# Kamino666/video_features

Hardware: AMD Instinct MI355X
Metric: frames/sec CLIP-ViT-B/32 uni_12 (higher is better)
Workload: dtype bf16; 1 GPU; model=CLIP-ViT-B/32, global_batch=256, seq_len=12, resolution=224, parallelism=dp1

## Files before the change

video_features_amd/models/clip_vit.py:

```python
from __future__ import annotations

from dataclasses import dataclass

import torch
from torch import nn

from .. import ops


@dataclass
class ViTConfig:
    input_resolution: int = 224
    patch_size: int = 32
    width: int = 768
    layers: int = 12
    heads: int = 12
    output_dim: int = 512


VIT_B32 = ViTConfig(patch_size=32)
VIT_B16 = ViTConfig(patch_size=16)


class LayerNorm(nn.LayerNorm):
    def forward(self, x: torch.Tensor) -> torch.Tensor:
        return ops.layer_norm(x, self.weight, self.bias, self.eps)


class MultiheadSelfAttention(nn.Module):
    def __init__(self, width: int, heads: int):
        super().__init__()
        self.heads = heads
        self.head_dim = width // heads
        self.qkv = nn.Linear(width, 3 * width)
        self.proj = nn.Linear(width, width)

    def forward(self, x: torch.Tensor) -> torch.Tensor:
        o = ops.mhsa_fused(self.qkv(x), self.heads)
        return self.proj(o)


class MLP(nn.Module):
    def __init__(self, width: int):
        super().__init__()
        self.c_fc = nn.Linear(width, 4 * width)
        self.c_proj = nn.Linear(4 * width, width)

    def forward(self, x: torch.Tensor) -> torch.Tensor:
        h = ops.linear_act(x, self.c_fc.weight, self.c_fc.bias, 'quick_gelu')
        return self.c_proj(h)


class ResidualAttentionBlock(nn.Module):
    def __init__(self, width: int, heads: int):
        super().__init__()
        self.ln_1 = LayerNorm(width)
        self.attn = MultiheadSelfAttention(width, heads)
        self.ln_2 = LayerNorm(width)
        self.mlp = MLP(width)

    def forward(self, x: torch.Tensor) -> torch.Tensor:
        x = x + self.attn(self.ln_1(x))
        x = x + self.mlp(self.ln_2(x))
        return x


class VisionTransformer(nn.Module):
    def __init__(self, cfg: ViTConfig = VIT_B32):
        super().__init__()
        self.cfg = cfg
        w = cfg.width
        self.conv1 = nn.Conv2d(3, w, kernel_size=cfg.patch_size,
                               stride=cfg.patch_size, bias=False)
        n_patches = (cfg.input_resolution // cfg.patch_size) ** 2
        scale = w ** -0.5
        self.class_embedding = nn.Parameter(scale * torch.randn(w))
        self.positional_embedding = nn.Parameter(
            scale * torch.randn(n_patches + 1, w))
        self.ln_pre = LayerNorm(w)
        self.blocks = nn.ModuleList(
            [ResidualAttentionBlock(w, cfg.heads) for _ in range(cfg.layers)])
        self.ln_post = LayerNorm(w)
        self.proj = nn.Parameter(scale * torch.randn(w, cfg.output_dim))

    def _patch_embed(self, x: torch.Tensor) -> torch.Tensor:
        if x.is_cuda:
            t = x.shape[0]
            p = self.cfg.patch_size
            g = x.shape[-1] // p
            xp = x.reshape(t, 3, g, p, g, p).permute(0, 2, 4, 1, 3, 5)
            xp = xp.reshape(t, g * g, 3 * p * p)
            w = self.conv1.weight.reshape(self.cfg.width, -1)
            return xp @ w.t()
        x = self.conv1(x)
        return x.flatten(2).transpose(1, 2)

    def forward(self, x: torch.Tensor) -> torch.Tensor:
        x = self._patch_embed(x)
        cls = self.class_embedding.to(x.dtype).expand(x.shape[0], 1, -1)
        x = torch.cat([cls, x], dim=1)
        x = x + self.positional_embedding.to(x.dtype)
        x = self.ln_pre(x)
        delta, res = None, x
        for blk in self.blocks:
            if delta is None:
                y1, s1 = blk.ln_1(res), res
            else:
                y1, s1 = ops.layer_norm_residual(delta, res, blk.ln_1.weight,
                                                 blk.ln_1.bias, blk.ln_1.eps)
            a = blk.attn(y1)
            y2, s2 = ops.layer_norm_residual(a, s1, blk.ln_2.weight,
                                             blk.ln_2.bias, blk.ln_2.eps)
            delta, res = blk.mlp(y2), s2
        x = delta + res
        x = self.ln_post(x[:, 0, :])
        return x @ self.proj.to(x.dtype)

    def encode_image(self, x: torch.Tensor) -> torch.Tensor:
        return self.forward(x)


def build_clip_vit(feature_type: str) -> VisionTransformer:
    if feature_type in ('CLIP-ViT-B/32', 'CLIP4CLIP-ViT-B-32'):
        return VisionTransformer(VIT_B32)
    if feature_type == 'CLIP-ViT-B/16':
        return VisionTransformer(VIT_B16)
    raise ValueError(f'unknown CLIP feature type {feature_type!r}')
```

video_features_amd/ops/__init__.py:

```python
from __future__ import annotations

import math
import os
from typing import Optional

import torch

_ext = None
_ext_err: Optional[str] = None


def _env_flag(name: str) -> bool:
    return os.environ.get(name, '').strip().lower() not in (
        '', '0', 'false', 'no', 'off')


def _load_extension():
    global _ext, _ext_err
    if _ext is not None or _ext_err is not None:
        return _ext
    try:
        from . import _vfa_hip
        _ext = _vfa_hip
    except ImportError as e:
        _ext_err = str(e)
    return _ext


def hip_available() -> bool:
    return _load_extension() is not None


def _use_hip(t: torch.Tensor) -> bool:
    if not t.is_cuda:
        return False
    if _env_flag('VFA_FORCE_TORCH_OPS'):
        return False
    ext = _load_extension()
    if ext is None:
        raise RuntimeError(
            'Tensor is on GPU but the VFA HIP extension is not built '
            f'(import error: {_ext_err}). Build it in-tree with '
            '`python setup.py build_ext --inplace` (PYTORCH_ROCM_ARCH=gfx950). '
            'Refusing to fall back to eager PyTorch on a GPU run.')
    return True


def layer_norm(x: torch.Tensor, weight: torch.Tensor, bias: torch.Tensor,
               eps: float = 1e-5) -> torch.Tensor:
    if _use_hip(x) and x.dtype in (torch.bfloat16, torch.float16, torch.float32):
        return _ext.layer_norm(x.contiguous(), weight, bias, eps)
    return torch.nn.functional.layer_norm(x, (x.shape[-1],), weight, bias, eps)


def quick_gelu(x: torch.Tensor) -> torch.Tensor:
    if _use_hip(x) and x.dtype in (torch.bfloat16, torch.float16, torch.float32):
        return _ext.quick_gelu(x.contiguous())
    return x * torch.sigmoid(1.702 * x)


def gelu(x: torch.Tensor) -> torch.Tensor:
    if _use_hip(x) and x.dtype in (torch.bfloat16, torch.float16, torch.float32):
        return _ext.gelu_tanh(x.contiguous())
    return torch.nn.functional.gelu(x, approximate='tanh')


def attention(q: torch.Tensor, k: torch.Tensor, v: torch.Tensor,
              scale: Optional[float] = None) -> torch.Tensor:
    if scale is None:
        scale = 1.0 / math.sqrt(q.shape[-1])
    if (_use_hip(q) and q.dtype in (torch.bfloat16, torch.float16, torch.float32)
            and q.shape[-2] <= 64 and q.shape[-1] <= 128):
        return _ext.mhsa(q.contiguous(), k.contiguous(), v.contiguous(),
                         float(scale))
    attn = (q @ k.transpose(-2, -1)) * scale
    attn = attn.softmax(dim=-1)
    return attn @ v


def layer_norm_residual(x: torch.Tensor, res: torch.Tensor,
                        weight: torch.Tensor, bias: torch.Tensor,
                        eps: float = 1e-5):
    if _use_hip(x) and x.dtype in (torch.bfloat16, torch.float16, torch.float32):
        y, s = _ext.layer_norm_residual(x.contiguous(), res.contiguous(),
                                        weight, bias, eps)
        return y, s
    s = x + res
    y = torch.nn.functional.layer_norm(s, (s.shape[-1],), weight, bias, eps)
    return y, s


def preprocess_u8_chw(frames_u8: torch.Tensor, mean, std,
                      bf16: bool = True) -> torch.Tensor:
    if _use_hip(frames_u8) and \
            (frames_u8.shape[1] * frames_u8.shape[2]) % 4 == 0:
        return _ext.u8_chw_norm(frames_u8.contiguous(), list(map(float, mean)),
                                list(map(float, std)), bf16)
    x = frames_u8.permute(0, 3, 1, 2).float() / 255.0
    mean_t = torch.as_tensor(mean, dtype=x.dtype, device=x.device)
    std_t = torch.as_tensor(std, dtype=x.dtype, device=x.device)
    x = (x - mean_t[:, None, None]) / std_t[:, None, None]
    return x.to(torch.bfloat16) if bf16 else x


def mhsa_fused(qkv: torch.Tensor, heads: int,
               scale: Optional[float] = None) -> torch.Tensor:
    b, n, three_e = qkv.shape
    e = three_e // 3
    d = e // heads
    if scale is None:
        scale = 1.0 / math.sqrt(d)
    if _use_hip(qkv) and qkv.dtype == torch.bfloat16 and d == 64:
        qkv5 = qkv.view(b, n, 3, heads, d)
        return _ext.flash_qkv(qkv5.contiguous(), float(scale))
    q, k, v = qkv.view(b, n, 3, heads, d).permute(2, 0, 3, 1, 4).unbind(0)
    o = attention(q.contiguous(), k.contiguous(), v.contiguous(), scale)
    return o.permute(0, 2, 1, 3).reshape(b, n, e)


def pwc_correlation(f1: torch.Tensor, f2: torch.Tensor,
                    max_disp: int = 4) -> torch.Tensor:
    if _use_hip(f1):
        return _ext.pwc_correlation(f1.contiguous(), f2.contiguous(), max_disp)
    return _pwc_correlation_torch(f1, f2, max_disp)


def _pwc_correlation_torch(f1: torch.Tensor, f2: torch.Tensor,
                           max_disp: int) -> torch.Tensor:
    b, c, h, w = f1.shape
    d = max_disp
    f2p = torch.nn.functional.pad(f2, (d, d, d, d))
    out = f1.new_empty(b, (2 * d + 1) ** 2, h, w)
    i = 0
    for dy in range(2 * d + 1):
        for dx in range(2 * d + 1):
            out[:, i] = (f1 * f2p[:, :, dy:dy + h, dx:dx + w]).mean(dim=1)
            i += 1
    return out


def bilinear_warp(x: torch.Tensor, flow: torch.Tensor) -> torch.Tensor:
    if _use_hip(x):
        return _ext.bilinear_warp(x.contiguous(), flow.contiguous())
    b, c, h, w = x.shape
    yy, xx = torch.meshgrid(
        torch.arange(h, device=x.device, dtype=x.dtype),
        torch.arange(w, device=x.device, dtype=x.dtype), indexing='ij')
    grid_x = (xx[None] + flow[:, 0]) / max(w - 1, 1) * 2 - 1
    grid_y = (yy[None] + flow[:, 1]) / max(h - 1, 1) * 2 - 1
    grid = torch.stack([grid_x, grid_y], dim=-1)
    warped = torch.nn.functional.grid_sample(x, grid, mode='bilinear',
                                             padding_mode='zeros',
                                             align_corners=True)
    mask = torch.nn.functional.grid_sample(torch.ones_like(x[:, :1]), grid,
                                           mode='bilinear', padding_mode='zeros',
                                           align_corners=True)
    return warped * (mask > 0.999).to(x.dtype)


def corr_lookup(pyramid, coords: torch.Tensor, radius: int = 4,
                nhwc: bool = False,
                out_dtype: Optional[torch.dtype] = None) -> torch.Tensor:
    if out_dtype is None:
        out_dtype = coords.dtype
    if _use_hip(coords) and radius == 4:
        return _ext.corr_lookup(list(pyramid), coords.contiguous(), nhwc,
                                out_dtype,
                                _env_flag('VFA_CORR_GMEM'))
    b, _, h, w = coords.shape
    r = radius
    cc = coords.permute(0, 2, 3, 1)
    out = []
    for lvl, corr in enumerate(pyramid):
        dx = torch.linspace(-r, r, 2 * r + 1, device=coords.device,
                            dtype=torch.float32)
        delta = torch.stack(torch.meshgrid(dx, dx, indexing='ij'), dim=-1)
        centroid = cc.reshape(b * h * w, 1, 1, 2) / (2 ** lvl)
        window = centroid + delta[None]
        sampled = grid_sample_bilinear(corr, window)
        out.append(sampled.reshape(b, h, w, -1))
    res = torch.cat(out, dim=-1).permute(0, 3, 1, 2).to(out_dtype)
    return res.contiguous(memory_format=torch.channels_last) if nhwc \
        else res.contiguous()


def convex_upsample(flow: torch.Tensor, mask: torch.Tensor,
                    nhwc: bool = False) -> torch.Tensor:
    if _use_hip(flow):
        return _ext.convex_upsample(flow, mask, nhwc)
    b, _, h, w = flow.shape
    m = (0.25 * mask.float()).view(b, 1, 9, 8, 8, h, w).softmax(dim=2)
    up = torch.nn.functional.unfold(8 * flow.float(), 3, padding=1)
    up = up.view(b, 2, 9, 1, 1, h, w)
    up = (m * up).sum(dim=2)
    return up.permute(0, 1, 4, 2, 5, 3).reshape(b, 2, 8 * h, 8 * w) \
        .to(flow.dtype)


def gru_zr(zr: torch.Tensor, hx: torch.Tensor, rhx: torch.Tensor,
           nhwc: bool = False) -> torch.Tensor:
    c = zr.shape[1] // 2
    if _use_hip(zr):
        return _ext.gru_zr(zr, hx, rhx, nhwc)
    z = torch.sigmoid(zr[:, :c])
    r = torch.sigmoid(zr[:, c:])
    rhx[:, :c] = r * hx[:, :c]
    return z


def gru_out(q: torch.Tensor, z: torch.Tensor, hx: torch.Tensor,
            nhwc: bool = False) -> None:
    if _use_hip(q):
        _ext.gru_out(q, z, hx, nhwc)
        return
    c = q.shape[1]
    hx[:, :c] = (1 - z) * hx[:, :c] + z * torch.tanh(q)


def instance_norm(x: torch.Tensor, eps: float = 1e-5, relu: bool = False,
                  nhwc: bool = False) -> torch.Tensor:
    if _use_hip(x):
        return _ext.instance_norm2d(x, eps, relu, nhwc)
    y = torch.nn.functional.instance_norm(x, eps=eps)
    return torch.nn.functional.relu(y) if relu else y


def maxpool3d_same(x: torch.Tensor, kernel, stride) -> torch.Tensor:
    def _pad1(n, k, s):
        total = max(k - s, 0) if n % s == 0 else max(k - (n % s), 0)
        return total // 2, total - total // 2

    t, h, w = x.shape[-3:]
    pt, ph, pw = _pad1(t, kernel[0], stride[0]), _pad1(h, kernel[1], stride[1]),         _pad1(w, kernel[2], stride[2])
    if _use_hip(x):
        out_sz = [(t + pt[0] + pt[1] - kernel[0]) // stride[0] + 1,
                  (h + ph[0] + ph[1] - kernel[1]) // stride[1] + 1,
                  (w + pw[0] + pw[1] - kernel[2]) // stride[2] + 1]
        return _ext.maxpool3d_same(x.contiguous(), list(kernel), list(stride),
                                   [pt[0], ph[0], pw[0]], out_sz)
    xp = torch.nn.functional.pad(
        x, (pw[0], pw[1], ph[0], ph[1], pt[0], pt[1]))
    return torch.nn.functional.max_pool3d(xp, tuple(kernel), tuple(stride))
# ... 258 lines not shown
```

video_features_amd/ops/csrc/bindings.cpp:

```cpp
#include <torch/extension.h>
#include <c10/hip/HIPStream.h>
#include <mutex>
#include <unordered_map>
#include <hip/hip_runtime.h>
#include <hip/hip_bf16.h>

extern "C" {
void vfa_quick_gelu(const void*, void*, long long, int, hipStream_t);
void vfa_gelu_tanh(const void*, void*, long long, int, hipStream_t);
void vfa_layer_norm(const void*, const void*, const void*, void*, long long,
                    int, float, int, hipStream_t);
void vfa_bilinear_warp(const void*, const void*, void*, int, int, int, int,
                       int, hipStream_t);
void vfa_grid_sample(const void*, const void*, void*, long long, int, int,
                     int, int, int, int, hipStream_t);
void vfa_corr_repack(const void*, void*, int, int, int, int, int,
                     hipStream_t);
void vfa_pwc_correlation(const void*, const void*, const void*, void*, int,
                         int, int, int, int, hipStream_t);
void vfa_mhsa_small(const void*, const void*, const void*, void*, int, int,
                    int, float, int, hipStream_t);
void vfa_flash_qkv(const void*, void*, int, int, int, float, hipStream_t);
void vfa_mfma_gemm16(const void*, const void*, void*, hipStream_t);
void vfa_layer_norm_residual(const void*, const void*, const void*,
                             const void*, void*, void*, long long, int,
                             float, int, hipStream_t);
void vfa_u8_chw_norm(const void*, void*, long long, int, int, const float*,
                     const float*, int, hipStream_t);
void vfa_corr_lookup(const void*, const void*, const void*, const void*,
                     const void*, void*, int, int, int, int, int, int, int,
                     int, int, long long, int, int, int, int, hipStream_t);
void vfa_convex_upsample(const void*, const void*, void*, int, int, int, int,
                         int, hipStream_t);
void vfa_gru_zr(const void*, const void*, void*, void*, int, int, int,
                long long, int, int, hipStream_t);
void vfa_gru_out(const void*, const void*, void*, int, int, int, long long,
                 int, int, hipStream_t);
void vfa_instance_norm2d(const void*, void*, int, int, int, float, int, int,
                         int, hipStream_t);
void vfa_maxpool3d_same(const void*, void*, long long, int, int, int, int,
                        int, int, int, int, int, int, int, int, int, int,
                        int, int, hipStream_t);
void vfa_maxpool2d_same(const void*, void*, long long, int, int, int, int,
                        int, int, int, int, int, int, int, int, int,
                        hipStream_t);
void vfa_linear_act(const void*, const void*, const void*, const void*,
                    void*, int, int, int, int, hipStream_t);
void vfa_temporal_merge(const void*, void*, int, int, int, int, int, int,
                        int, long long, int, int, hipStream_t);
void vfa_conv2d_nhwc(const void*, const void*, const void*, const void*,
                     const void*, void*, int, int, int, int, int, int, int,
                     int, int, int, int, int, int, int, int, hipStream_t);
void vfa_pad2d_nhwc(const void*, void*, int, int, int, int, int, int, int,
                    int, int, hipStream_t);
void vfa_avgpool2d_nhwc(const void*, void*, long long, int, int, int, int,
                        int, int, hipStream_t);
void vfa_attnpool_tokens(const void*, const void*, void*, long long, int, int,
                         hipStream_t);
void vfa_attention_pool_d64(const void*, const void*, void*, long long, int,
                            int, float, hipStream_t);
}

namespace {

int dtype_tag(const torch::Tensor& t) {
  switch (t.scalar_type()) {
    case torch::kFloat32: return 0;
    case torch::kBFloat16: return 1;
    case torch::kFloat16: return 2;
    default:
      TORCH_CHECK(false, "unsupported dtype ", t.scalar_type());
  }
}

hipStream_t current_stream() {
  return c10::hip::getCurrentHIPStream().stream();
}

torch::Tensor quick_gelu(torch::Tensor x) {
  TORCH_CHECK(x.is_cuda() && x.is_contiguous());
  auto out = torch::empty_like(x);
  vfa_quick_gelu(x.data_ptr(), out.data_ptr(), x.numel(), dtype_tag(x),
                 current_stream());
  return out;
}

torch::Tensor gelu_tanh(torch::Tensor x) {
  TORCH_CHECK(x.is_cuda() && x.is_contiguous());
  auto out = torch::empty_like(x);
  vfa_gelu_tanh(x.data_ptr(), out.data_ptr(), x.numel(), dtype_tag(x),
                current_stream());
  return out;
}

torch::Tensor layer_norm(torch::Tensor x, torch::Tensor w, torch::Tensor b,
                         double eps) {
  TORCH_CHECK(x.is_cuda() && x.is_contiguous());
  const int d = (int)x.size(-1);
  TORCH_CHECK(w.numel() == d && b.numel() == d, "affine shape mismatch");
  auto wc = w.contiguous().to(x.scalar_type());
  auto bc = b.contiguous().to(x.scalar_type());
  auto out = torch::empty_like(x);
  vfa_layer_norm(x.data_ptr(), wc.data_ptr(), bc.data_ptr(), out.data_ptr(),
                 x.numel() / d, d, (float)eps, dtype_tag(x), current_stream());
  return out;
}

torch::Tensor bilinear_warp(torch::Tensor x, torch::Tensor flow) {
  TORCH_CHECK(x.is_cuda() && x.is_contiguous() && flow.is_contiguous());
  TORCH_CHECK(x.dim() == 4 && flow.dim() == 4 && flow.size(1) == 2);
  auto flow_c = flow.to(x.scalar_type()).contiguous();
  auto out = torch::empty_like(x);
  vfa_bilinear_warp(x.data_ptr(), flow_c.data_ptr(), out.data_ptr(),
                    (int)x.size(0), (int)x.size(1), (int)x.size(2),
                    (int)x.size(3), dtype_tag(x), current_stream());
  return out;
}

torch::Tensor grid_sample_bilinear(torch::Tensor x, torch::Tensor coords) {
  TORCH_CHECK(x.is_cuda() && x.is_contiguous());
  TORCH_CHECK(coords.dim() == 4 && coords.size(-1) == 2);
  TORCH_CHECK(coords.size(0) == x.size(0));
  auto cc = coords.to(x.scalar_type()).contiguous();
  const long long n = x.size(0);
  const int c = (int)x.size(1), h = (int)x.size(2), w = (int)x.size(3);
  const int ho = (int)coords.size(1), wo = (int)coords.size(2);
  auto out = torch::empty({(long)n, c, ho, wo}, x.options());
  vfa_grid_sample(x.data_ptr(), cc.data_ptr(), out.data_ptr(), n, c, h, w, ho,
                  wo, dtype_tag(x), current_stream());
  return out;
}

torch::Tensor pwc_correlation(torch::Tensor f1, torch::Tensor f2,
                              int64_t max_disp) {
  TORCH_CHECK(f1.is_cuda() && f1.is_contiguous() && f2.is_contiguous());
  TORCH_CHECK(max_disp == 4, "kernel is specialized for max_disp=4");
  TORCH_CHECK(f1.sizes() == f2.sizes());
  TORCH_CHECK(f1.size(1) <= 256,
              "corr_wave registers cover C<=256 (PWC max is 196)");
  const int b = (int)f1.size(0), c = (int)f1.size(1);
  const int h = (int)f1.size(2), w = (int)f1.size(3);
  auto opts = f1.options();
  auto f1p = torch::empty({b, h + 8, w + 8, c}, opts);
  auto f2p = torch::empty({b, h + 8, w + 8, c}, opts);
  const int tag = dtype_tag(f1);
  auto stream = current_stream();
  if (c > 64) vfa_corr_repack(f1.data_ptr(), f1p.data_ptr(), b, c, h, w, tag, stream);
  vfa_corr_repack(f2.data_ptr(), f2p.data_ptr(), b, c, h, w, tag, stream);
  auto out = torch::empty({b, 81, h, w}, opts.dtype(torch::kFloat32));
  vfa_pwc_correlation(f1.data_ptr(), f1p.data_ptr(), f2p.data_ptr(),
                      out.data_ptr(), b, c, h, w, tag, stream);
  return out.to(f1.scalar_type());
}

torch::Tensor mhsa(torch::Tensor q, torch::Tensor k, torch::Tensor v,
                   double scale) {
  TORCH_CHECK(q.is_cuda() && q.is_contiguous() && k.is_contiguous() &&
              v.is_contiguous());
  TORCH_CHECK(q.dim() == 4);
  const int n = (int)q.size(2), d = (int)q.size(3);
  TORCH_CHECK(n <= 64 && d <= 128, "mhsa kernel covers N<=64, D<=128");
  const int bh = (int)(q.size(0) * q.size(1));
  auto out = torch::empty_like(q);
  vfa_mhsa_small(q.data_ptr(), k.data_ptr(), v.data_ptr(), out.data_ptr(), bh,
                 n, d, (float)scale, dtype_tag(q), current_stream());
  return out;
}

std::vector<torch::Tensor> layer_norm_residual(torch::Tensor x,
                                               torch::Tensor res,
                                               torch::Tensor w,
                                               torch::Tensor b, double eps) {
  TORCH_CHECK(x.is_cuda() && x.is_contiguous() && res.is_contiguous());
  TORCH_CHECK(x.sizes() == res.sizes());
  const int d = (int)x.size(-1);
  auto wc = w.contiguous().to(x.scalar_type());
  auto bc = b.contiguous().to(x.scalar_type());
  auto y = torch::empty_like(x);
  auto s = torch::empty_like(x);
  vfa_layer_norm_residual(x.data_ptr(), res.data_ptr(), wc.data_ptr(),
                          bc.data_ptr(), y.data_ptr(), s.data_ptr(),
                          x.numel() / d, d, (float)eps, dtype_tag(x),
                          current_stream());
  return {y, s};
}

torch::Tensor u8_chw_norm(torch::Tensor frames, std::vector<double> mean,
                          std::vector<double> std_, bool bf16) {
  TORCH_CHECK(frames.is_cuda() && frames.is_contiguous());
  TORCH_CHECK(frames.scalar_type() == torch::kUInt8);
  TORCH_CHECK(frames.dim() == 4 && frames.size(3) == 3, "(T,H,W,3) expected");
  const long long t = frames.size(0);
  const int h = (int)frames.size(1), w = (int)frames.size(2);
  TORCH_CHECK((h * w) % 4 == 0);
  float m[3] = {(float)mean[0], (float)mean[1], (float)mean[2]};
  float s[3] = {(float)std_[0], (float)std_[1], (float)std_[2]};
  auto out = torch::empty({(long)t, 3, h, w},
                          frames.options().dtype(bf16 ? torch::kBFloat16
                                                      : torch::kFloat32));
  vfa_u8_chw_norm(frames.data_ptr(), out.data_ptr(), t, h, w, m, s,
                  bf16 ? 1 : 0, current_stream());
  return out;
}

torch::Tensor flash_qkv(torch::Tensor qkv, double scale) {
  TORCH_CHECK(qkv.is_cuda() && qkv.is_contiguous() && qkv.dim() == 5);
  TORCH_CHECK(qkv.size(2) == 3 && qkv.size(4) == 64,
              "flash_qkv covers head_dim 64");
  TORCH_CHECK(qkv.scalar_type() == torch::kBFloat16);
  const int b = (int)qkv.size(0), n = (int)qkv.size(1);
  const int h = (int)qkv.size(3);
  auto out = torch::empty({b, n, h * 64L}, qkv.options());
  vfa_flash_qkv(qkv.data_ptr(), out.data_ptr(), b, n, h, (float)scale,
                current_stream());
  return out;
}

torch::Tensor mfma_gemm16(torch::Tensor a, torch::Tensor b) {
  TORCH_CHECK(a.is_cuda() && a.is_contiguous() && b.is_contiguous());
  TORCH_CHECK(a.sizes() == torch::IntArrayRef({16, 32}) &&
              b.sizes() == torch::IntArrayRef({32, 16}));
  auto af = a.to(torch::kFloat32), bf = b.to(torch::kFloat32);
  auto d = torch::empty({16, 16}, af.options());
  vfa_mfma_gemm16(af.data_ptr(), bf.data_ptr(), d.data_ptr(),
                  current_stream());
  return d;
}

torch::Tensor corr_lookup(std::vector<torch::Tensor> pyramid,
                          torch::Tensor coords, bool nhwc,
                          torch::ScalarType out_dtype, bool force_gmem) {
  const int levels = (int)pyramid.size();
  TORCH_CHECK(levels >= 1 && levels <= 4, "1..4 pyramid levels");
  TORCH_CHECK(coords.is_cuda() && coords.dim() == 4 && coords.size(1) == 2);
  auto cc = coords.to(torch::kFloat32).contiguous();
  const long long b = coords.size(0);
  const int h = (int)coords.size(2), w = (int)coords.size(3);
  const long long npix = b * h * w;
  int hs[4] = {1, 1, 1, 1}, ws[4] = {1, 1, 1, 1};
  const void* ptrs[4] = {nullptr, nullptr, nullptr, nullptr};
  long long lds_floats = 0;
  for (int l = 0; l < levels; ++l) {
    auto& t = pyramid[l];
    TORCH_CHECK(t.is_cuda() && t.is_contiguous() &&
                t.scalar_type() == torch::kFloat32);
    TORCH_CHECK(t.size(0) == npix && t.size(1) == 1, "plane-per-pixel");
    hs[l] = (int)t.size(2);
    ws[l] = (int)t.size(3);
    ptrs[l] = t.data_ptr();
    lds_floats += hs[l] * ws[l];
  }
  for (int l = levels; l < 4; ++l) ptrs[l] = ptrs[levels - 1];
  const int ctot = levels * 81;
  auto opts = coords.options().dtype(out_dtype);
  torch::Tensor out;
  if (nhwc) {
    out = torch::empty({b, h, w, ctot}, opts)
// ... 169 lines not shown
  TORCH_CHECK(x.scalar_type() == torch::kBFloat16 &&
              w.scalar_type() == torch::kBFloat16);
  const int b = (int)x.size(0), c = (int)x.size(1);
  const int h = (int)x.size(2), ww = (int)x.size(3);
  const int kout = (int)w.size(0), kh = (int)w.size(2), kw = (int)w.size(3);
  const int c8 = (c + 7) / 8 * 8;
  TORCH_CHECK(w.size(1) == c8, "weight C must be input C padded up to 8");
  const int hp = h + (int)(pt + pb), wp = ww + (int)(pl + pr);
  const int oh = (hp - kh) / (int)stride_h + 1;
  const int ow = (wp - kw) / (int)stride_w + 1;
  auto stream = current_stream();
  const bool inline_pad = (c8 == c);
  torch::Tensor xp = x;
  if (!inline_pad && (pt > 0 || pb > 0 || pl > 0 || pr > 0 || c8 != c)) {
    xp = torch::empty({b, hp, wp, c8}, x.options());
    vfa_pad2d_nhwc(x.data_ptr(), xp.data_ptr(), b, h, ww, c, c8, (int)pt,
                   (int)pb, (int)pl, (int)pr, stream);
    xp = xp.permute({0, 3, 1, 2});
  }
  static std::unordered_map<int, torch::Tensor> zpages;
  static std::mutex zp_mu;
  torch::Tensor zpage;
  {
    std::lock_guard<std::mutex> lk(zp_mu);
    auto it = zpages.find((int)x.get_device());
    if (it == zpages.end()) {
      zpage = torch::zeros({512}, x.options());
      zpages.emplace((int)x.get_device(), zpage);
    } else {
      zpage = it->second;
    }
  }
  const void* bptr = nullptr;
  torch::Tensor bc;
  if (bias.has_value()) {
    bc = bias->contiguous().to(torch::kBFloat16);
    TORCH_CHECK(bc.numel() == kout);
    bptr = bc.data_ptr();
  }
  const void* rptr = nullptr;
  if (res.has_value()) {
    TORCH_CHECK(cl_contig(*res) && res->scalar_type() == torch::kBFloat16 &&
                res->numel() == (long long)b * oh * ow * kout,
                "residual must be CL bf16 of the output shape");
    rptr = res->data_ptr();
  }
  torch::Tensor out;
  int ldc = kout;
  void* optr;
  if (out_buf.has_value()) {
    out = *out_buf;
    TORCH_CHECK(cl_contig(out) && out.scalar_type() == torch::kBFloat16 &&
                out.size(0) == b && out.size(2) == oh && out.size(3) == ow &&
                out_off + kout <= out.size(1),
                "out buffer must be CL bf16 (B, >=off+kout, OH, OW)");
    ldc = (int)out.size(1);
    optr = static_cast<char*>(out.data_ptr()) + out_off * 2;
  } else {
    out = torch::empty({(long)b, oh, ow, kout}, x.options())
              .permute({0, 3, 1, 2});
    optr = out.data_ptr();
  }
  if (inline_pad)
    vfa_conv2d_nhwc(xp.data_ptr(), w.data_ptr(), bptr, rptr,
                    zpage.data_ptr(), optr, b, h, ww, c8, oh, ow,
                    kout, kh, kw, (int)stride_h, (int)stride_w, (int)pt,
                    (int)pl, ldc, (int)act, stream);
  else
    vfa_conv2d_nhwc(xp.data_ptr(), w.data_ptr(), bptr, rptr,
                    zpage.data_ptr(), optr, b, hp, wp, c8, oh,
                    ow, kout, kh, kw, (int)stride_h, (int)stride_w, 0, 0,
                    ldc, (int)act, stream);
  return out;
}

torch::Tensor temporal_merge(torch::Tensor y, int64_t b, int64_t kt,
                             int64_t st, int64_t p0, int64_t p1,
                             bool relu) {
  TORCH_CHECK(y.is_cuda() && y.dim() == 4);
  TORCH_CHECK(cl_contig(y), "channels_last expected");
  const int bt = (int)y.size(0), cin = (int)y.size(1);
  const int h = (int)y.size(2), w = (int)y.size(3);
  const int o = cin / (int)kt, t = bt / (int)b;
  const int to = (int)((t + p0 + p1 - kt) / st + 1);
  auto out = torch::empty({(long)b * to, h, w, o}, y.options())
                 .permute({0, 3, 1, 2});
  vfa_temporal_merge(y.data_ptr(), out.data_ptr(), (int)b, t, to, (int)kt,
                     (int)st, (int)p0, o, (long long)h * w, relu ? 1 : 0,
                     dtype_tag(y), current_stream());
  return out;
}

torch::Tensor avgpool2d_nhwc(torch::Tensor x, int64_t k) {
  TORCH_CHECK(x.is_cuda() && x.dim() == 4 && cl_contig(x),
              "x must be channels_last");
  TORCH_CHECK(x.scalar_type() == torch::kBFloat16, "avgpool2d_nhwc: bf16");
  TORCH_CHECK(x.size(1) % 8 == 0, "avgpool2d_nhwc: C % 8 == 0 required");
  TORCH_CHECK(k >= 1 && k <= x.size(2) && k <= x.size(3),
              "avgpool2d_nhwc: window larger than the input");
  const int64_t oh = x.size(2) / k, ow = x.size(3) / k;
  auto out = torch::empty({x.size(0), oh, ow, x.size(1)}, x.options())
                 .permute({0, 3, 1, 2});
  vfa_avgpool2d_nhwc(x.data_ptr(), out.data_ptr(), x.size(0), (int)x.size(1),
                     (int)x.size(2), (int)x.size(3), (int)oh, (int)ow, (int)k,
                     current_stream());
  return out;
}

torch::Tensor attnpool_tokens(torch::Tensor x, torch::Tensor pos) {
  TORCH_CHECK(x.is_cuda() && x.dim() == 3 && x.is_contiguous());
  TORCH_CHECK(pos.is_cuda() && pos.dim() == 2 && pos.is_contiguous());
  TORCH_CHECK(x.scalar_type() == torch::kBFloat16 &&
              pos.scalar_type() == torch::kBFloat16, "attnpool_tokens: bf16");
  const int64_t hw = x.size(1), c = x.size(2);
  TORCH_CHECK(hw >= 1 && c % 8 == 0, "attnpool_tokens: C % 8 == 0 required");
  TORCH_CHECK(pos.size(0) == hw + 1 && pos.size(1) == c,
              "positional embedding must be (HW+1, C)");
  auto t = torch::empty({x.size(0), hw + 1, c}, x.options());
  vfa_attnpool_tokens(x.data_ptr(), pos.data_ptr(), t.data_ptr(), x.size(0),
                      (int)hw, (int)c, current_stream());
  return t;
}

torch::Tensor attention_pool(torch::Tensor q, torch::Tensor kv,
                             int64_t heads) {
  TORCH_CHECK(q.is_cuda() && q.dim() == 2 && q.is_contiguous());
  TORCH_CHECK(kv.is_cuda() && kv.dim() == 3 && kv.is_contiguous());
  TORCH_CHECK(q.scalar_type() == torch::kBFloat16 &&
              kv.scalar_type() == torch::kBFloat16, "attention_pool: bf16");
  const int64_t b = q.size(0), c = q.size(1), l = kv.size(1);
  TORCH_CHECK(heads >= 1 && c == heads * 64,
              "attention_pool covers head_dim 64");
  TORCH_CHECK(kv.size(0) == b && kv.size(2) == 2 * c && l >= 1,
              "kv must be (B, L>=1, 2C)");
  auto out = torch::empty({b, c}, q.options());
  vfa_attention_pool_d64(q.data_ptr(), kv.data_ptr(), out.data_ptr(), b,
                         (int)heads, (int)l, 0.125f, current_stream());
  return out;
}

}

PYBIND11_MODULE(TORCH_EXTENSION_NAME, m) {
  m.def("quick_gelu", &quick_gelu);
  m.def("gelu_tanh", &gelu_tanh);
  m.def("layer_norm", &layer_norm);
  m.def("bilinear_warp", &bilinear_warp);
  m.def("grid_sample_bilinear", &grid_sample_bilinear);
  m.def("pwc_correlation", &pwc_correlation);
  m.def("mhsa", &mhsa);
  m.def("flash_qkv", &flash_qkv);
  m.def("mfma_gemm16", &mfma_gemm16);
  m.def("layer_norm_residual", &layer_norm_residual);
  m.def("u8_chw_norm", &u8_chw_norm);
  m.def("corr_lookup", &corr_lookup);
  m.def("convex_upsample", &convex_upsample);
  m.def("gru_zr", &gru_zr);
  m.def("gru_out", &gru_out);
  m.def("instance_norm2d", &instance_norm2d);
  m.def("maxpool3d_same", &maxpool3d_same);
  m.def("maxpool2d_same", &maxpool2d_same);
  m.def("linear_act", &linear_act);
  m.def("conv2d_nhwc", &conv2d_nhwc);
  m.def("temporal_merge", &temporal_merge);
  m.def("avgpool2d_nhwc", &avgpool2d_nhwc);
  m.def("attnpool_tokens", &attnpool_tokens);
  m.def("attention_pool", &attention_pool);
  m.attr("gfx_arch") = "gfx950";
}
```

video_features_amd/ops/csrc/layernorm.hip:

```cpp
#include "vfa_common.h"

namespace {

template <typename T>
__global__ void layernorm_kernel(const T* __restrict__ in,
                                 const T* __restrict__ weight,
                                 const T* __restrict__ bias,
                                 T* __restrict__ out, int rows, int d,
                                 float eps) {
  constexpr int VEC = 16 / sizeof(T);
  __shared__ float red[2][8];
  const int row = blockIdx.x;
  if (row >= rows) return;
  const T* x = in + (long long)row * d;
  T* y = out + (long long)row * d;
  const int tid = threadIdx.x;
  const int lane = tid & 63, wave = tid >> 6;
  const int nwaves = blockDim.x >> 6;

  float sum = 0.f, sumsq = 0.f;
  using VecT = __attribute__((ext_vector_type(4))) unsigned;
  const int dvec = d / VEC;
  for (int i = tid; i < dvec; i += blockDim.x) {
    T tmp[VEC];
// ... 102 lines not shown
    float mean = s / d;
    red[0][0] = mean;
    red[1][0] = rsqrtf(ss / d - mean * mean + eps);
  }
  __syncthreads();
  const float mean = red[0][0], rstd = red[1][0];
  for (int i = tid; i < dvec; i += blockDim.x) {
    T tx[VEC], tw[VEC], tb[VEC];
    *reinterpret_cast<VecT*>(tx) =
        *reinterpret_cast<const VecT*>(sr + (long long)i * VEC);
    *reinterpret_cast<VecT*>(tw) =
        *reinterpret_cast<const VecT*>(weight + (long long)i * VEC);
    *reinterpret_cast<VecT*>(tb) =
        *reinterpret_cast<const VecT*>(bias + (long long)i * VEC);
#pragma unroll
    for (int j = 0; j < VEC; ++j) {
      float v = (to_f32<T>(tx[j]) - mean) * rstd;
      tx[j] = from_f32<T>(v * to_f32<T>(tw[j]) + to_f32<T>(tb[j]));
    }
    *reinterpret_cast<VecT*>(yr + (long long)i * VEC) =
        *reinterpret_cast<VecT*>(tx);
  }
  for (int i = dvec * VEC + tid; i < d; i += blockDim.x) {
    float v = (to_f32<T>(sr[i]) - mean) * rstd;
    yr[i] = from_f32<T>(v * to_f32<T>(weight[i]) + to_f32<T>(bias[i]));
  }
}

template <typename T>
__global__ void layernorm_wave_kernel(const T* __restrict__ in,
                                      const T* __restrict__ weight,
                                      const T* __restrict__ bias,
                                      T* __restrict__ out, long long rows,
                                      int d, float eps) {
  constexpr int VEC = 16 / sizeof(T);
  const long long row = (long long)blockIdx.x * 4 + (threadIdx.x >> 6);
  if (row >= rows) return;
  const int lane = threadIdx.x & 63;
  const T* x = in + row * d;
  T* y = out + row * d;
  using VecT = __attribute__((ext_vector_type(4))) unsigned;
  const int dvec = d / VEC;
  float sum = 0.f, sumsq = 0.f;
  for (int i = lane; i < dvec; i += 64) {
    T tmp[VEC];
    *reinterpret_cast<VecT*>(tmp) =
        *reinterpret_cast<const VecT*>(x + (long long)i * VEC);
#pragma unroll
    for (int j = 0; j < VEC; ++j) {
      float v = to_f32<T>(tmp[j]);
      sum += v;
      sumsq += v * v;
    }
  }
  for (int i = dvec * VEC + lane; i < d; i += 64) {
    float v = to_f32<T>(x[i]);
    sum += v;
    sumsq += v * v;
  }
  sum = wave_allreduce_sum(sum);
  sumsq = wave_allreduce_sum(sumsq);
  const float mean = sum / d;
  const float rstd = rsqrtf(sumsq / d - mean * mean + eps);
  for (int i = lane; i < dvec; i += 64) {
    T tx[VEC], tw[VEC], tb[VEC];
    *reinterpret_cast<VecT*>(tx) =
        *reinterpret_cast<const VecT*>(x + (long long)i * VEC);
    *reinterpret_cast<VecT*>(tw) =
        *reinterpret_cast<const VecT*>(weight + (long long)i * VEC);
    *reinterpret_cast<VecT*>(tb) =
        *reinterpret_cast<const VecT*>(bias + (long long)i * VEC);
#pragma unroll
    for (int j = 0; j < VEC; ++j) {
      float v = (to_f32<T>(tx[j]) - mean) * rstd;
      tx[j] = from_f32<T>(v * to_f32<T>(tw[j]) + to_f32<T>(tb[j]));
    }
    *reinterpret_cast<VecT*>(y + (long long)i * VEC) =
        *reinterpret_cast<VecT*>(tx);
  }
  for (int i = dvec * VEC + lane; i < d; i += 64) {
    float v = (to_f32<T>(x[i]) - mean) * rstd;
    y[i] = from_f32<T>(v * to_f32<T>(weight[i]) + to_f32<T>(bias[i]));
  }
}

template <typename T>
__global__ void layernorm_res_wave_kernel(const T* __restrict__ x,
                                          const T* __restrict__ res,
                                          const T* __restrict__ weight,
                                          const T* __restrict__ bias,
                                          T* __restrict__ y,
                                          T* __restrict__ s_out,
                                          long long rows, int d, float eps) {
  constexpr int VEC = 16 / sizeof(T);
  const long long row = (long long)blockIdx.x * 4 + (threadIdx.x >> 6);
  if (row >= rows) return;
  const int lane = threadIdx.x & 63;
  const T* xr = x + row * d;
  const T* rr = res + row * d;
  T* sr = s_out + row * d;
  T* yr = y + row * d;
  using VecT = __attribute__((ext_vector_type(4))) unsigned;
  const int dvec = d / VEC;
  float sum = 0.f, sumsq = 0.f;
  for (int i = lane; i < dvec; i += 64) {
    T tx[VEC], tr[VEC];
    *reinterpret_cast<VecT*>(tx) =
        *reinterpret_cast<const VecT*>(xr + (long long)i * VEC);
    *reinterpret_cast<VecT*>(tr) =
        *reinterpret_cast<const VecT*>(rr + (long long)i * VEC);
#pragma unroll
    for (int j = 0; j < VEC; ++j) {
      float v = to_f32<T>(tx[j]) + to_f32<T>(tr[j]);
      tx[j] = from_f32<T>(v);
      sum += v;
      sumsq += v * v;
    }
    *reinterpret_cast<VecT*>(sr + (long long)i * VEC) =
        *reinterpret_cast<VecT*>(tx);
  }
  for (int i = dvec * VEC + lane; i < d; i += 64) {
    float v = to_f32<T>(xr[i]) + to_f32<T>(rr[i]);
    sr[i] = from_f32<T>(v);
    sum += v;
    sumsq += v * v;
  }
  sum = wave_allreduce_sum(sum);
  sumsq = wave_allreduce_sum(sumsq);
  const float mean = sum / d;
  const float rstd = rsqrtf(sumsq / d - mean * mean + eps);
  for (int i = lane; i < dvec; i += 64) {
    T tx[VEC], tw[VEC], tb[VEC];
    *reinterpret_cast<VecT*>(tx) =
        *reinterpret_cast<const VecT*>(sr + (long long)i * VEC);
    *reinterpret_cast<VecT*>(tw) =
        *reinterpret_cast<const VecT*>(weight + (long long)i * VEC);
    *reinterpret_cast<VecT*>(tb) =
        *reinterpret_cast<const VecT*>(bias + (long long)i * VEC);
#pragma unroll
    for (int j = 0; j < VEC; ++j) {
      float v = (to_f32<T>(tx[j]) - mean) * rstd;
      tx[j] = from_f32<T>(v * to_f32<T>(tw[j]) + to_f32<T>(tb[j]));
    }
    *reinterpret_cast<VecT*>(yr + (long long)i * VEC) =
        *reinterpret_cast<VecT*>(tx);
  }
  for (int i = dvec * VEC + lane; i < d; i += 64) {
    float v = (to_f32<T>(sr[i]) - mean) * rstd;
    yr[i] = from_f32<T>(v * to_f32<T>(weight[i]) + to_f32<T>(bias[i]));
  }
}

template <typename T>
void launch_ln(const void* in, const void* w, const void* b, void* out,
               long long rows, int d, float eps, hipStream_t stream) {
  if (d <= 4096) {
    const unsigned grid = (unsigned)((rows + 3) / 4);
    hipLaunchKernelGGL((layernorm_wave_kernel<T>), dim3(grid), dim3(256), 0,
                       stream, (const T*)in, (const T*)w, (const T*)b,
                       (T*)out, rows, d, eps);
    return;
  }
  int block = d >= 2048 ? 512 : 256;
  hipLaunchKernelGGL((layernorm_kernel<T>), dim3((unsigned)rows), dim3(block),
                     0, stream, (const T*)in, (const T*)w, (const T*)b,
                     (T*)out, (int)rows, d, eps);
}

}

extern "C" void vfa_layer_norm(const void* in, const void* w, const void* b,
                               void* out, long long rows, int d, float eps,
                               int dtype, hipStream_t stream) {
  switch (dtype) {
    case VFA_F32: launch_ln<float>(in, w, b, out, rows, d, eps, stream); break;
    case VFA_BF16:
      launch_ln<__hip_bfloat16>(in, w, b, out, rows, d, eps, stream); break;
    case VFA_F16: launch_ln<__half>(in, w, b, out, rows, d, eps, stream); break;
  }
}

extern "C" void vfa_layer_norm_residual(const void* x, const void* res,
                                        const void* w, const void* b,
                                        void* y, void* s_out, long long rows,
                                        int d, float eps, int dtype,
                                        hipStream_t stream) {
  if (d <= 4096) {
    const unsigned grid = (unsigned)((rows + 3) / 4);
    switch (dtype) {
      case VFA_F32:
        hipLaunchKernelGGL((layernorm_res_wave_kernel<float>), dim3(grid),
                           dim3(256), 0, stream, (const float*)x,
                           (const float*)res, (const float*)w,
                           (const float*)b, (float*)y, (float*)s_out, rows,
                           d, eps);
        break;
      case VFA_BF16:
        hipLaunchKernelGGL((layernorm_res_wave_kernel<__hip_bfloat16>),
                           dim3(grid), dim3(256), 0, stream,
                           (const __hip_bfloat16*)x,
                           (const __hip_bfloat16*)res,
                           (const __hip_bfloat16*)w, (const __hip_bfloat16*)b,
                           (__hip_bfloat16*)y, (__hip_bfloat16*)s_out, rows,
                           d, eps);
        break;
      case VFA_F16:
        hipLaunchKernelGGL((layernorm_res_wave_kernel<__half>), dim3(grid),
                           dim3(256), 0, stream, (const __half*)x,
                           (const __half*)res, (const __half*)w,
                           (const __half*)b, (__half*)y, (__half*)s_out,
                           rows, d, eps);
        break;
    }
    return;
  }
  int block = d >= 2048 ? 512 : 256;
  switch (dtype) {
    case VFA_F32:
      hipLaunchKernelGGL((layernorm_res_kernel<float>), dim3((unsigned)rows),
                         dim3(block), 0, stream, (const float*)x,
                         (const float*)res, (const float*)w, (const float*)b,
                         (float*)y, (float*)s_out, (int)rows, d, eps);
      break;
    case VFA_BF16:
      hipLaunchKernelGGL((layernorm_res_kernel<__hip_bfloat16>),
                         dim3((unsigned)rows), dim3(block), 0, stream,
                         (const __hip_bfloat16*)x, (const __hip_bfloat16*)res,
                         (const __hip_bfloat16*)w, (const __hip_bfloat16*)b,
                         (__hip_bfloat16*)y, (__hip_bfloat16*)s_out,
                         (int)rows, d, eps);
      break;
    case VFA_F16:
      hipLaunchKernelGGL((layernorm_res_kernel<__half>), dim3((unsigned)rows),
                         dim3(block), 0, stream, (const __half*)x,
                         (const __half*)res, (const __half*)w,
                         (const __half*)b, (__half*)y, (__half*)s_out,
                         (int)rows, d, eps);
      break;
  }
}
```

Before: 80330 frames/sec.

## Compute only CLS token in final ViT block and fuse embedding with ln_pre

The final transformer block now computes queries, attention, MLP and residual only for the CLS token, since only that token reaches the output. Keys and values are still computed for all tokens and attention is done with an attention_pool kernel. A new fused kernel also combines the class-token concat, positional embedding add and ln_pre LayerNorm into one pass, removing several elementwise launches and intermediate tensors. An environment flag can restore the full-tail path.

```diff
diff --git a/video_features_amd/models/clip_vit.py b/video_features_amd/models/clip_vit.py
--- a/video_features_amd/models/clip_vit.py
+++ b/video_features_amd/models/clip_vit.py
@@ -1,8 +1,10 @@
 from __future__ import annotations
 
 from dataclasses import dataclass
+from typing import Optional
 
 import torch
+import torch.nn.functional as F
 from torch import nn
 
 from .. import ops
@@ -97,12 +99,12 @@
 
     def forward(self, x: torch.Tensor) -> torch.Tensor:
         x = self._patch_embed(x)
-        cls = self.class_embedding.to(x.dtype).expand(x.shape[0], 1, -1)
-        x = torch.cat([cls, x], dim=1)
-        x = x + self.positional_embedding.to(x.dtype)
-        x = self.ln_pre(x)
+        x = ops.clip_embed_ln(x, self.class_embedding,
+                              self.positional_embedding, self.ln_pre.weight,
+                              self.ln_pre.bias, self.ln_pre.eps)
+        full_tail = ops._env_flag('VFA_CLIP_FULL_TAIL')
         delta, res = None, x
-        for blk in self.blocks:
+        for blk in (self.blocks if full_tail else self.blocks[:-1]):
             if delta is None:
                 y1, s1 = blk.ln_1(res), res
             else:
@@ -112,9 +114,33 @@
             y2, s2 = ops.layer_norm_residual(a, s1, blk.ln_2.weight,
                                              blk.ln_2.bias, blk.ln_2.eps)
             delta, res = blk.mlp(y2), s2
-        x = delta + res
-        x = self.ln_post(x[:, 0, :])
+        if full_tail:
+            x = delta + res
+            x = self.ln_post(x[:, 0, :])
+        else:
+            x = self._cls_tail(self.blocks[-1], delta, res)
         return x @ self.proj.to(x.dtype)
+
+    def _cls_tail(self, blk: ResidualAttentionBlock,
+                  delta: Optional[torch.Tensor],
+                  res: torch.Tensor) -> torch.Tensor:
+        w = self.cfg.width
+        if delta is None:
+            y1, s1 = blk.ln_1(res), res
+        else:
+            y1, s1 = ops.layer_norm_residual(delta, res, blk.ln_1.weight,
+                                             blk.ln_1.bias, blk.ln_1.eps)
+        qkv = blk.attn.qkv
+        kv = F.linear(y1, qkv.weight[w:], qkv.bias[w:])
+        q = F.linear(y1[:, 0], qkv.weight[:w], qkv.bias[:w])
+        o = ops.attention_pool(q, kv, blk.attn.heads)
+        a = blk.attn.proj(o)
+        y2, s2 = ops.layer_norm_residual(a, s1[:, 0], blk.ln_2.weight,
+                                         blk.ln_2.bias, blk.ln_2.eps)
+        d = blk.mlp(y2)
+        y, _ = ops.layer_norm_residual(d, s2, self.ln_post.weight,
+                                       self.ln_post.bias, self.ln_post.eps)
+        return y
 
     def encode_image(self, x: torch.Tensor) -> torch.Tensor:
         return self.forward(x)
diff --git a/video_features_amd/ops/__init__.py b/video_features_amd/ops/__init__.py
--- a/video_features_amd/ops/__init__.py
+++ b/video_features_amd/ops/__init__.py
@@ -88,6 +88,18 @@
     s = x + res
     y = torch.nn.functional.layer_norm(s, (s.shape[-1],), weight, bias, eps)
     return y, s
+
+
+def clip_embed_ln(pe: torch.Tensor, cls: torch.Tensor, pos: torch.Tensor,
+                  weight: torch.Tensor, bias: torch.Tensor,
+                  eps: float = 1e-5) -> torch.Tensor:
+    if (_use_hip(pe) and pe.shape[-1] % 8 == 0
+            and pe.dtype in (torch.bfloat16, torch.float16, torch.float32)):
+        return _ext.clip_embed_ln(pe.contiguous(), cls, pos, weight, bias,
+                                  eps)
+    c = cls.to(pe.dtype).expand(pe.shape[0], 1, -1)
+    x = torch.cat([c, pe], dim=1) + pos.to(pe.dtype)
+    return layer_norm(x, weight, bias, eps)
 
 
 def preprocess_u8_chw(frames_u8: torch.Tensor, mean, std,
diff --git a/video_features_amd/ops/csrc/bindings.cpp b/video_features_amd/ops/csrc/bindings.cpp
--- a/video_features_amd/ops/csrc/bindings.cpp
+++ b/video_features_amd/ops/csrc/bindings.cpp
@@ -59,6 +59,9 @@
                          hipStream_t);
 void vfa_attention_pool_d64(const void*, const void*, void*, long long, int,
                             int, float, hipStream_t);
+void vfa_clip_embed_ln(const void*, const void*, const void*, const void*,
+                       const void*, void*, long long, int, int, float, int,
+                       hipStream_t);
 }
 
 namespace {
@@ -103,6 +106,29 @@
   auto out = torch::empty_like(x);
   vfa_layer_norm(x.data_ptr(), wc.data_ptr(), bc.data_ptr(), out.data_ptr(),
                  x.numel() / d, d, (float)eps, dtype_tag(x), current_stream());
+  return out;
+}
+
+torch::Tensor clip_embed_ln(torch::Tensor pe, torch::Tensor cls,
+                            torch::Tensor pos, torch::Tensor w,
+                            torch::Tensor b, double eps) {
+  TORCH_CHECK(pe.is_cuda() && pe.is_contiguous() && pe.dim() == 3,
+              "clip_embed_ln: pe must be a contiguous (T, P, W) GPU tensor");
+  const long long t = pe.size(0);
+  const int p = (int)pe.size(1), d = (int)pe.size(2);
+  TORCH_CHECK(d % 8 == 0, "clip_embed_ln: W % 8 == 0 required");
+  TORCH_CHECK(cls.numel() == d && w.numel() == d && b.numel() == d &&
+                  pos.dim() == 2 && pos.size(0) == p + 1 && pos.size(1) == d,
+              "clip_embed_ln: shape mismatch");
+  auto cc = cls.contiguous().to(pe.scalar_type());
+  auto pc = pos.contiguous().to(pe.scalar_type());
+  auto wc = w.contiguous().to(pe.scalar_type());
+  auto bc = b.contiguous().to(pe.scalar_type());
+  auto out = torch::empty({(long)t, p + 1, d}, pe.options());
+  vfa_clip_embed_ln(pe.data_ptr(), cc.data_ptr(), pc.data_ptr(),
+                    wc.data_ptr(), bc.data_ptr(), out.data_ptr(),
+                    t * (p + 1), p, d, (float)eps, dtype_tag(pe),
+                    current_stream());
   return out;
 }
 
@@ -578,6 +604,7 @@
   m.def("flash_qkv", &flash_qkv);
   m.def("mfma_gemm16", &mfma_gemm16);
   m.def("layer_norm_residual", &layer_norm_residual);
+  m.def("clip_embed_ln", &clip_embed_ln);
   m.def("u8_chw_norm", &u8_chw_norm);
   m.def("corr_lookup", &corr_lookup);
   m.def("convex_upsample", &convex_upsample);
diff --git a/video_features_amd/ops/csrc/layernorm.hip b/video_features_amd/ops/csrc/layernorm.hip
--- a/video_features_amd/ops/csrc/layernorm.hip
+++ b/video_features_amd/ops/csrc/layernorm.hip
@@ -278,6 +278,74 @@
 }
 
 template <typename T>
+__global__ void clip_embed_ln_kernel(const T* __restrict__ pe,
+                                     const T* __restrict__ cls,
+                                     const T* __restrict__ pos,
+                                     const T* __restrict__ weight,
+                                     const T* __restrict__ bias,
+                                     T* __restrict__ out, long long rows,
+                                     int p, int d, float eps) {
+  constexpr int VEC = 16 / sizeof(T);
+  const long long row = (long long)blockIdx.x * 4 + (threadIdx.x >> 6);
+  if (row >= rows) return;
+  const int lane = threadIdx.x & 63;
+  const long long t = row / (p + 1);
+  const int j = (int)(row % (p + 1));
+  const T* x = j == 0 ? cls : pe + (t * p + (j - 1)) * d;
+  const T* pj = pos + (long long)j * d;
+  T* y = out + row * d;
+  using VecT = __attribute__((ext_vector_type(4))) unsigned;
+  const int dvec = d / VEC;
+  float sum = 0.f, sumsq = 0.f;
+  for (int i = lane; i < dvec; i += 64) {
+    T tx[VEC], tp[VEC];
+    *reinterpret_cast<VecT*>(tx) =
+        *reinterpret_cast<const VecT*>(x + (long long)i * VEC);
+    *reinterpret_cast<VecT*>(tp) =
+        *reinterpret_cast<const VecT*>(pj + (long long)i * VEC);
+#pragma unroll
+    for (int e = 0; e < VEC; ++e) {
+      float v = to_f32<T>(tx[e]) + to_f32<T>(tp[e]);
+      sum += v;
+      sumsq += v * v;
+    }
+  }
+  sum = wave_allreduce_sum(sum);
+  sumsq = wave_allreduce_sum(sumsq);
+  const float mean = sum / d;
+  const float rstd = rsqrtf(sumsq / d - mean * mean + eps);
+  for (int i = lane; i < dvec; i += 64) {
+    T tx[VEC], tp[VEC], tw[VEC], tb[VEC];
+    *reinterpret_cast<VecT*>(tx) =
+        *reinterpret_cast<const VecT*>(x + (long long)i * VEC);
+    *reinterpret_cast<VecT*>(tp) =
+        *reinterpret_cast<const VecT*>(pj + (long long)i * VEC);
+    *reinterpret_cast<VecT*>(tw) =
+        *reinterpret_cast<const VecT*>(weight + (long long)i * VEC);
+    *reinterpret_cast<VecT*>(tb) =
+        *reinterpret_cast<const VecT*>(bias + (long long)i * VEC);
+#pragma unroll
+    for (int e = 0; e < VEC; ++e) {
+      float v = (to_f32<T>(tx[e]) + to_f32<T>(tp[e]) - mean) * rstd;
+      tx[e] = from_f32<T>(v * to_f32<T>(tw[e]) + to_f32<T>(tb[e]));
+    }
+    *reinterpret_cast<VecT*>(y + (long long)i * VEC) =
+        *reinterpret_cast<VecT*>(tx);
+  }
+}
+
+template <typename T>
+void launch_clip_embed_ln(const void* pe, const void* cls, const void* pos,
+                          const void* w, const void* b, void* out,
+                          long long rows, int p, int d, float eps,
+                          hipStream_t stream) {
+  const unsigned grid = (unsigned)((rows + 3) / 4);
+  hipLaunchKernelGGL((clip_embed_ln_kernel<T>), dim3(grid), dim3(256), 0,
+                     stream, (const T*)pe, (const T*)cls, (const T*)pos,
+                     (const T*)w, (const T*)b, (T*)out, rows, p, d, eps);
+}
+
+template <typename T>
 void launch_ln(const void* in, const void* w, const void* b, void* out,
                long long rows, int d, float eps, hipStream_t stream) {
   if (d <= 4096) {
@@ -303,6 +371,28 @@
     case VFA_BF16:
       launch_ln<__hip_bfloat16>(in, w, b, out, rows, d, eps, stream); break;
     case VFA_F16: launch_ln<__half>(in, w, b, out, rows, d, eps, stream); break;
+  }
+}
+
+extern "C" void vfa_clip_embed_ln(const void* pe, const void* cls,
+                                  const void* pos, const void* w,
+                                  const void* b, void* out, long long rows,
+                                  int p, int d, float eps, int dtype,
+                                  hipStream_t stream) {
+  if (rows <= 0) return;
+  switch (dtype) {
+    case VFA_F32:
+      launch_clip_embed_ln<float>(pe, cls, pos, w, b, out, rows, p, d, eps,
+                                  stream);
+      break;
+    case VFA_BF16:
+      launch_clip_embed_ln<__hip_bfloat16>(pe, cls, pos, w, b, out, rows, p,
+                                           d, eps, stream);
+      break;
+    case VFA_F16:
+      launch_clip_embed_ln<__half>(pe, cls, pos, w, b, out, rows, p, d, eps,
+                                   stream);
+      break;
   }
 }
 
```

Result: faster. 84720 frames/sec (median of 6 runs) (+5.5%).
